# lisqzqng/Video-based-gait-analysis-for-dementia

Hardware: AMD Instinct MI355X
Metric: frames/sec (224x224, seq=16) (higher is better)
Workload: dtype f32

## Files before the change

### video-based-gait-analysis-for-dementia_amd/csrc/conv_pw.hip

```cpp
#include "kernels.h"
#include "device.h"

namespace grk {

namespace {


template <int KC, int NT, int RUN , bool MASK >
__global__ __launch_bounds__(256) __attribute__((amdgpu_waves_per_eu(2))) void conv_pw_f32(const ConvArgs a) {
    constexpr int run = RUN;
    constexpr int KS = KC / 4;
    const int lane = threadIdx.x & 63, l15 = lane & 15, lq = lane >> 4;
    const int HW = a.H * a.W, runs = HW / (16 * run), groups = (a.Cout + 16 * NT - 1) / (16 * NT);
    const int w = blockIdx.x * 4 + (threadIdx.x >> 6);
    if (w >= a.N * runs * groups) return;
    const int g = w % groups, t = w / groups, n = t / runs, px0 = (t - n * runs) * 16 * run, co0 = g * 16 * NT;
    float bw[KS][NT];
#pragma unroll
    for (int s = 0; s < KS; ++s)
#pragma unroll
        for (int nt = 0; nt < NT; ++nt) bw[s][nt] = a.w[(size_t)(4 * s + lq) * a.CoutPad + co0 + nt * 16 + l15];
    float bias[NT];
#pragma unroll
    for (int nt = 0; nt < NT; ++nt) bias[nt] = a.bias[co0 + nt * 16 + l15];
    const float* inp = a.in + ((size_t)n * a.in_ctot + a.in_coff + lq) * HW + px0 + l15;
    float* outp = a.out + ((size_t)n * a.out_ctot + a.out_coff + co0 + l15) * HW + px0 + 4 * lq;
    const float* addp = a.n_add ? a.add[0] + ((size_t)n * a.add_ctot[0] + a.add_coff[0] + co0 + l15) * HW + px0 + 4 * lq : nullptr;
    const size_t cstr = (size_t)16 * HW;
    float cur[KS], nxt[KS];
#pragma unroll
    for (int s = 0; s < KS; ++s) cur[s] = inp[(size_t)(4 * s) * HW];
    for (int tile = 0; tile < run; ++tile) {
        const int tn = tile + 1 < run ? tile + 1 : tile;
        f32x4 res[NT];
        if (addp) {
#pragma unroll
            for (int nt = 0; nt < NT; ++nt)
                if (!MASK || co0 + nt * 16 + l15 < a.Cout) res[nt] = *reinterpret_cast<const f32x4*>(addp + nt * cstr + 16 * tile);
        }
#pragma unroll
        for (int s = 0; s < KS; ++s) nxt[s] = inp[(size_t)(4 * s) * HW + 16 * tn];
        f32x4 acc[NT];
#pragma unroll
        for (int nt = 0; nt < NT; ++nt) acc[nt] = f32x4{0.f, 0.f, 0.f, 0.f};
#pragma unroll
        for (int s = 0; s < KS; ++s)
#pragma unroll
            for (int nt = 0; nt < NT; ++nt) acc[nt] = __builtin_amdgcn_mfma_f32_16x16x4f32(cur[s], bw[s][nt], acc[nt], 0, 0, 0);
#pragma unroll
        for (int nt = 0; nt < NT; ++nt) {
            f32x4 v = acc[nt] + bias[nt];
            if (addp) v += res[nt];
            if (a.relu) {
#pragma unroll
                for (int r = 0; r < 4; ++r) v[r] = fmaxf(v[r], 0.f);
            }
            if (!MASK || co0 + nt * 16 + l15 < a.Cout) *reinterpret_cast<f32x4*>(outp + nt * cstr + 16 * tile) = v;
        }
#pragma unroll
        for (int s = 0; s < KS; ++s) cur[s] = nxt[s];
    }
}

}

bool conv_pw_eligible(int cin, int cout, int ks, int stride, int h, int w, int n_add) {
    return ks == 1 && stride == 1 && n_add <= 1 && (h * w) % (16 * 14) == 0 && ((cin == 64 && cout >= 17) || (cin == 128 && cout >= 17 && cout <= 32));
}

hipError_t launch_conv_pw(ConvArgs a, hipStream_t s) {
    if (!conv_pw_eligible(a.Cin, a.Cout, a.ks, a.stride, a.H, a.W, a.n_add) || (a.n_add == 1 && a.add_shift[0] != 0) || a.CinPad < a.Cin)
        return hipErrorInvalidValue;
    const int nt = a.Cout > 32 ? 4 : 2, groups = (a.Cout + 16 * nt - 1) / (16 * nt), tiles = a.H * a.W / 16;
    if (a.CoutPad < groups * 16 * nt) return hipErrorInvalidValue;
    if (tiles % 14 != 0 || tiles % 2 != 0) return hipErrorInvalidValue;
    const bool lng = (long)a.N * (tiles / 14) * groups >= 800;
    const dim3 grid((a.N * (tiles / (lng ? 14 : 2)) * groups + 3) / 4);
    const bool mask = a.Cout % (16 * nt) != 0;
#define GRK_PW2(KC, NT, RUN) (mask ? launch_k(conv_pw_f32<KC, NT, RUN, true>, grid, dim3(256), 0, s, a) : launch_k(conv_pw_f32<KC, NT, RUN, false>, grid, dim3(256), 0, s, a))
#define GRK_PW(KC, NT) (lng ? GRK_PW2(KC, NT, 14) : GRK_PW2(KC, NT, 2))
    if (a.Cin == 64) return nt == 4 ? GRK_PW(64, 4) : GRK_PW(64, 2);
    return GRK_PW(128, 2);
#undef GRK_PW2
#undef GRK_PW
}

}
```

### video-based-gait-analysis-for-dementia_amd/csrc/conv_stem.hip

```cpp
#include "kernels.h"
#include "device.h"

namespace grk {

namespace {

__global__ __launch_bounds__(256) void conv_stem_f32(const ConvArgs a) {
    const int lane = threadIdx.x & 63, l15 = lane & 15, lq = lane >> 4;
    const int row = blockIdx.x * 4 + (threadIdx.x >> 6);
    if (row >= a.N * a.Ho) return;
    const int n = row / a.Ho, y = row - n * a.Ho;
    const float* w = a.w;
    float bw[7][4];
#pragma unroll
    for (int s = 0; s < 7; ++s)
#pragma unroll
        for (int nt = 0; nt < 4; ++nt) bw[s][nt] = w[(s * 4 + nt) * 64 + lane];
    float bias[4];
#pragma unroll
    for (int nt = 0; nt < 4; ++nt) bias[nt] = a.bias[nt * 16 + l15];
    const float* rowp[7];
    int kxm1[7];
    bool yok[7];
    const float* inb = a.in + ((size_t)n * a.in_ctot + a.in_coff) * a.H * a.W;
#pragma unroll
    for (int s = 0; s < 7; ++s) {
        const int k = 4 * s + lq, kk = k < 27 ? k : 26, c = kk / 9, t = kk - 9 * c, ky = t / 3, kx = t - 3 * ky;
        const int yin = 2 * y + ky - 1;
        yok[s] = yin >= 0 && yin < a.H;
        rowp[s] = inb + ((size_t)c * a.H + (yok[s] ? yin : 0)) * a.W;
        kxm1[s] = kx - 1;
    }
    auto fetch = [&](int x0, float (&v)[7]) {
#pragma unroll
        for (int s = 0; s < 7; ++s) {
            const int xi = 2 * (x0 + l15) + kxm1[s];
            const bool ok = yok[s] && xi >= 0 && xi < a.W;
            const float t = rowp[s][ok ? xi : 0];
            v[s] = ok ? t : 0.f;
        }
    };
    float cur[7], nxt[7];
    fetch(0, cur);
    float* ob = a.out + (((size_t)n * a.out_ctot + a.out_coff + l15) * a.Ho + y) * a.Wo + 4 * lq;
    const size_t cstride = (size_t)16 * a.Ho * a.Wo;
    for (int x0 = 0; x0 < a.Wo; x0 += 16) {
        fetch(x0 + 16 < a.Wo ? x0 + 16 : x0, nxt);
        f32x4 acc[4];
#pragma unroll
        for (int nt = 0; nt < 4; ++nt) acc[nt] = f32x4{0.f, 0.f, 0.f, 0.f};
#pragma unroll
        for (int s = 0; s < 7; ++s)
#pragma unroll
            for (int nt = 0; nt < 4; ++nt) acc[nt] = __builtin_amdgcn_mfma_f32_16x16x4f32(cur[s], bw[s][nt], acc[nt], 0, 0, 0);
#pragma unroll
        for (int nt = 0; nt < 4; ++nt) {
            f32x4 v = acc[nt] + bias[nt];
            if (a.relu) {
#pragma unroll
                for (int r = 0; r < 4; ++r) v[r] = fmaxf(v[r], 0.f);
            }
            *reinterpret_cast<f32x4*>(ob + nt * cstride + x0) = v;
        }
#pragma unroll
        for (int s = 0; s < 7; ++s) cur[s] = nxt[s];
    }
}

}

bool conv_stem_eligible(int cin, int cout, int ks, int stride, int h, int w, int n_add) {
    return cin == 3 && cout == 64 && ks == 3 && stride == 2 && n_add == 0 && h % 2 == 0 && w % 32 == 0;
}

void pack_stem_weights(const double* w_folded , float* out ) {
    for (int s = 0; s < 7; ++s)
        for (int nt = 0; nt < 4; ++nt)
            for (int lq = 0; lq < 4; ++lq)
                for (int l15 = 0; l15 < 16; ++l15) {
                    const int k = 4 * s + lq, co = 16 * nt + l15;
                    out[(s * 4 + nt) * 64 + lq * 16 + l15] = k < 27 ? (float)w_folded[(size_t)co * 27 + k] : 0.f;
                }
}

hipError_t launch_conv_stem(ConvArgs a, hipStream_t s) {
    if (!conv_stem_eligible(a.Cin, a.Cout, a.ks, a.stride, a.H, a.W, a.n_add) || a.Ho * 2 != a.H || a.Wo * 2 != a.W) return hipErrorInvalidValue;
    const int rows = a.N * a.Ho;
    return launch_k(conv_stem_f32, dim3((rows + 3) / 4), dim3(256), 0, s, a);
}

}
```

### video-based-gait-analysis-for-dementia_amd/csrc/grnet_run.cpp

```cpp
#include "grnet_impl.h"

namespace grk { thread_local GraphRecorder* g_recorder = nullptr; }

int grnet::allocate() {
    if (plan_arena(compact, arena_plan)) return fail(GRNET_ESTATE, "the activation arena could not be planned: a launch group or the assignment violates the sharing rule");
    const size_t total = (size_t)arena_plan.total;
    arena_floats = total;
    void* q = nullptr;
    if (hipMalloc(&q, total * sizeof(float)) != hipSuccess)
        return fail(GRNET_ENOMEM, std::string("hipMalloc of the ") + (compact ? "compact " : "") + "activation arena (" + std::to_string(total * 4 >> 20) + " MiB) failed");
    arena = static_cast<float*>(q);
    if (hipMemset(arena, 0, 64 * sizeof(float)) != hipSuccess) return fail(GRNET_EHIP, "hipMemset failed");
    zeros = arena;
    if (hipEventCreateWithFlags(&ev_fork, hipEventDisableTiming) != hipSuccess) return fail(GRNET_EHIP, "hipEventCreate failed");
    if (int rc = install_schedule(max_frames)) return rc;
    if (hipStreamCreateWithFlags(&capture_stream, hipStreamNonBlocking) != hipSuccess) return fail(GRNET_EHIP, "hipStreamCreate failed");
    const size_t n = max_frames;
    int rc;
    if ((rc = dev_alloc(&d_plf, n * 128 * 24))) return rc;
    if ((rc = dev_alloc(&d_csf, n * 64 * 24))) return rc;
    if ((rc = dev_alloc(&d_stats, softmax_pool_ws_floats((int)n)))) return rc;
    if ((rc = dev_alloc(&d_rot6d, n * 144))) return rc;
    if ((rc = dev_alloc(&d_shape, n * 10))) return rc;
    if ((rc = dev_alloc(&d_cam, n * 3))) return rc;
// ... 258 lines not shown
            src.w = fp.w_dev[i][j - i - 1];
        }
    }
    HIP_TRY(dtype == 1 ? launch_hr_fuse_up_bf16(a, s) : launch_hr_fuse_up(a, s));
    return 0;
}

grnet::HeadOutputs grnet::head_outputs(const grnet_outputs_t& o) const {
    return {o.pred_rot6d ? o.pred_rot6d : d_rot6d, o.rotmat ? o.rotmat : d_rotmat, o.theta ? o.theta : d_theta,
            o.verts ? o.verts : d_verts,           o.kp_3d ? o.kp_3d : d_kp3d,     o.kp_2d ? o.kp_2d : d_kp2d};
}

int grnet::enqueue(const float* frames, int n, const grnet_outputs_t& o, hipStream_t s, bool convs_only) {
    int launches = 0;
    last_n = n;
    float* plf = o.point_local_feat ? o.point_local_feat : d_plf;
    float* csf = o.cam_shape_feats ? o.cam_shape_feats : d_csf;
    const auto [rot6d, rotmat, theta, verts, kp3d, kp2d] = head_outputs(o);
    const std::vector<Op>& ops = ops_flat;
    const std::vector<hipEvent_t>& op_events = op_events_flat;
    GraphRecorder* rec = g_recorder;
    const bool lanes = multi_lane && !rec;
    std::vector<hipGraphNode_t> lane_last(kLanes, nullptr), op_node(rec ? ops.size() : 0, nullptr);
    hipStream_t lane_stream[kLanes];
    for (int l = 0; l < kLanes; ++l) lane_stream[l] = s;
    if (lanes) {
        HIP_TRY(hipEventRecord(ev_fork, s));
        for (int l = 1; l < lanes_used; ++l) {
            lane_stream[l] = side[l];
            HIP_TRY(hipStreamWaitEvent(side[l], ev_fork, 0));
        }
    }
    hipStream_t caller = s;
    for (size_t oi = 0; oi < ops.size(); ++oi) {
        const Op& op = ops[oi];
        if (convs_only && op.kind != Op::CONV && op.kind != Op::FUSEUP) continue;
        s = lane_stream[op.lane];
        const int lane = multi_lane ? op.lane : 0;
        if (lanes)
            for (int w : op.waits) HIP_TRY(hipStreamWaitEvent(s, op_events[w], 0));
        if (tl_start && !rec) HIP_TRY(hipEventRecord((*tl_start)[oi], s));
        if (rec) {
            rec->deps.clear();
            rec->n_chain = lane_last[lane] ? 1 : 0;
            if (lane_last[lane]) rec->deps.push_back(lane_last[lane]);
            if (multi_lane)
                for (int w : op.waits)
                    if (op_node[w] && std::find(rec->deps.begin(), rec->deps.end(), op_node[w]) == rec->deps.end()) rec->deps.push_back(op_node[w]);
        }
        static const char* abl_skip = GRNET_AB_STR(ABL_SKIP);
        if (abl_skip && (op.kind == Op::CONV || op.kind == Op::FUSEUP)) {
            const std::string lbl = op_label(op);
            bool skip = false;
            for (const char* q = abl_skip; *q;) {
                const char* e = strchr(q, ',');
                const std::string pat = e ? std::string(q, e) : std::string(q);
                if (!pat.empty() && lbl.find(pat) != std::string::npos) skip = true;
                q = e ? e + 1 : q + strlen(q);
            }
            if (skip) {
                if (tl_end && !rec) HIP_TRY(hipEventRecord((*tl_end)[oi], s));
                if (lanes && op.record) HIP_TRY(hipEventRecord(op_events[oi], s));
                continue;
            }
        }
        switch (op.kind) {
// ... 9 lines not shown
            }
            case Op::SUM: {
                const auto& sv = sum_views[op.conv_idx];
                SumArgs a = op.sum;
                a.N = n;
                bind(sv.out, a.out, a.out_ctot, a.out_coff);
                for (int k = 0; k < a.n_add; ++k) {
                    bind(sv.adds[k].v, a.add[k], a.add_ctot[k], a.add_coff[k]);
                    a.add_shift[k] = sv.adds[k].shift;
                }
                if (dtype == 1) HIP_TRY(launch_fuse_sum_bf16(a, s));
                else HIP_TRY(launch_fuse_sum(a, s));
                ++launches;
                break;
            }
            case Op::FUSEUP:
                if (int rc = launch_fuse_up_op(fuse_ups[op.conv_idx], n, s)) return rc;
                ++launches;
                break;
            case Op::BILINEAR:
                if (dtype == 1) HIP_TRY(launch_bilinear2x_bf16(base(op.bin), base(op.bout), n, op.bin.c, op.bin.h, op.bin.w, s));
                else HIP_TRY(launch_bilinear2x(base(op.bin), base(op.bout), n, op.bin.c, op.bin.h, op.bin.w, s));
                ++launches;
                break;
            case Op::POOL:
                if (dtype == 1)
                    HIP_TRY(launch_softmax_pool_bf16(base(v_heat), v_heat.ctot, bf16_at(v_smpl_feats), 128, v_smpl_feats.ctot, bf16_at(v_csmap), 64,
                                                     v_csmap.ctot, d_stats, n, 56 * 56, s));
                else
                    HIP_TRY(launch_softmax_pool(base(v_heat), 25, base(v_smpl_feats), 128, base(v_csmap), 64, plf, csf, d_stats, n, 56 * 56, s));
                ++launches;
                break;
            case Op::TAIL:
                HIP_TRY(launch_head_tail(d_stats, true, plf, csf, tailw, rot6d, d_shape, d_cam, rotmat, theta, n, s));
                ++launches;
                break;
            case Op::SMPL:
                HIP_TRY(launch_smpl(d_shape, rotmat, d_cam, smpl, d_A, verts, kp3d, kp2d, n, s));
                launches += 4;
                break;
        }
        if (tl_end && !rec) HIP_TRY(hipEventRecord((*tl_end)[oi], s));
        if (lanes && op.record) HIP_TRY(hipEventRecord(op_events[oi], s));
        if (rec && !rec->deps.empty()) lane_last[lane] = op_node[oi] = rec->deps[0];
    }
    s = caller;
    if (lanes)
        for (int l = 1; l < lanes_used; ++l) {
            HIP_TRY(hipEventRecord(ev_join[l], side[l]));
            HIP_TRY(hipStreamWaitEvent(s, ev_join[l], 0));
        }
    if (!convs_only) {
        auto copy_out = [&](float* dst, const float* src, size_t bytes) -> int {
            if (!dst) return 0;
            if (!rec) { HIP_TRY(hipMemcpyAsync(dst, src, bytes, hipMemcpyDeviceToDevice, s)); return 0; }
            std::vector<hipGraphNode_t> deps;
            for (hipGraphNode_t nd : lane_last) if (nd) deps.push_back(nd);
            hipGraphNode_t node = nullptr;
            HIP_TRY(hipGraphAddMemcpyNode1D(&node, rec->graph, deps.data(), deps.size(), dst, src, bytes, hipMemcpyDeviceToDevice));
            return 0;
        };
        int rc;
        if (dtype == 1) {
            auto conv_out = [&](float* dst, const View& v) -> int {
                if (!dst) return 0;
                if (rec) {
                    rec->deps.clear();
                    for (hipGraphNode_t nd : lane_last) if (nd) rec->deps.push_back(nd);
                }
                HIP_TRY(launch_nhwc_bf16_to_nchw_f32(base(v), dst, n, v.c, v.h, v.w, v.ctot, v.coff, s));
                return 0;
            };
// ... 297 lines not shown
```

### video-based-gait-analysis-for-dementia_amd/csrc/head_kernels.hip

```cpp
#include "kernels.h"
#include "device.h"

namespace grk {

__global__ __launch_bounds__(256) void fuse_sum_kernel(const SumArgs a) {
    const int HW = a.H * a.W, n = blockIdx.x / a.C, c = blockIdx.x - n * a.C;
    const float inv_w = 1.0f / (float)a.W;
    for (int pix = threadIdx.x * 4; pix < HW; pix += 1024) {
        f32x4 v = f32x4{0.f, 0.f, 0.f, 0.f};
        for (int k = 0; k < a.n_add; ++k) {
            const int sh = a.add_shift[k];
            if (sh == 0) {
                v += *reinterpret_cast<const f32x4*>(a.add[k] + ((size_t)n * a.add_ctot[k] + a.add_coff[k] + c) * HW + pix);
            } else {
                const int hs = a.H >> sh, ws = a.W >> sh;
                const float* ap = a.add[k] + ((size_t)n * a.add_ctot[k] + a.add_coff[k] + c) * (hs * ws);
#pragma unroll
                for (int r = 0; r < 4; ++r) {
                    const int y = (int)(((float)(pix + r) + 0.5f) * inv_w), x = (pix + r) - y * a.W;
                    v[r] += ap[(y >> sh) * ws + (x >> sh)];
                }
            }
        }
        if (a.relu) {
// ... 286 lines not shown
    const float ux = a2x - d * b1x, uy = a2y - d * b1y, uz = a2z - d * b1z;
    const float n2 = fmaxf(sqrtf(ux * ux + uy * uy + uz * uz), 1e-6f);
    const float b2x = ux / n2, b2y = uy / n2, b2z = uz / n2;
    const float b3x = b1y * b2z - b1z * b2y, b3y = b1z * b2x - b1x * b2z, b3z = b1x * b2y - b1y * b2x;
    R[0] = b1x; R[1] = b2x; R[2] = b3x;
    R[3] = b1y; R[4] = b2y; R[5] = b3y;
    R[6] = b1z; R[7] = b2z; R[8] = b3z;
}

__device__ __forceinline__ void rotmat_to_aa_dev(const float* R, float* aa) {
    const float m00 = R[0], m01 = R[3], m02 = R[6];
    const float m10 = R[1], m11 = R[4], m12 = R[7];
    const float m20 = R[2], m21 = R[5], m22 = R[8];
    float q0, q1, q2, q3, t;
    if (m22 < 1e-6f) {
        if (m00 > m11) { t = 1.f + m00 - m11 - m22; q0 = m12 - m21; q1 = t; q2 = m01 + m10; q3 = m20 + m02; }
        else           { t = 1.f - m00 + m11 - m22; q0 = m20 - m02; q1 = m01 + m10; q2 = t; q3 = m12 + m21; }
    } else {
        if (m00 < -m11) { t = 1.f - m00 - m11 + m22; q0 = m01 - m10; q1 = m20 + m02; q2 = m12 + m21; q3 = t; }
        else            { t = 1.f + m00 + m11 + m22; q0 = t; q1 = m12 - m21; q2 = m20 - m02; q3 = m01 - m10; }
    }
    const float sc = 0.5f / sqrtf(t);
    q0 *= sc; q1 *= sc; q2 *= sc; q3 *= sc;
    const float s2 = q1 * q1 + q2 * q2 + q3 * q3;
    const float sn = sqrtf(s2);
    const float two_theta = 2.f * (q0 < 0.f ? atan2f(-sn, -q0) : atan2f(sn, q0));
    const float k = s2 > 0.f ? two_theta / sn : 2.f;
    float a0 = q1 * k, a1 = q2 * k, a2 = q3 * k;
    aa[0] = isnan(a0) ? 0.f : a0;
    aa[1] = isnan(a1) ? 0.f : a1;
    aa[2] = isnan(a2) ? 0.f : a2;
}

template <bool FROM_PARTS>
__global__ __launch_bounds__(256) void head_tail_kernel(const float* __restrict__ part, const float* __restrict__ zstats, float* __restrict__ plf, float* __restrict__ csf, TailWeights w,
                                                          float* __restrict__ rot6d, float* __restrict__ shape,
                                                          float* __restrict__ cam, float* __restrict__ rotmat,
                                                          float* __restrict__ theta) {
    __shared__ float s_plf[128 * 24];
    __shared__ __align__(16) float s_csf[64 * 24];
    __shared__ float s_pose[24 * 6];
    __shared__ float s_sc[13];
    __shared__ float s_pp[4][144];
    __shared__ float s_sp[13][8];
    __shared__ float s_zw[kPoolSplit + 1][24];
    const int n = blockIdx.x, tid = threadIdx.x;
    if constexpr (FROM_PARTS) {
        if (tid < 24) {
            float m[kPoolSplit], sm[kPoolSplit], M = -INFINITY, S = 0.f;
#pragma unroll
            for (int z = 0; z < kPoolSplit; ++z) {
                m[z] = zstats ? zstats[(((size_t)n * kPoolSplit + z) * 24 + tid) * 2] : 0.f;
                sm[z] = zstats ? zstats[(((size_t)n * kPoolSplit + z) * 24 + tid) * 2 + 1] : 0.f;
                M = fmaxf(M, m[z]);
            }
#pragma unroll
            for (int z = 0; z < kPoolSplit; ++z) {
                const float wz = zstats ? expf(m[z] - M) : 1.f;
                s_zw[z][tid] = wz;
                S += sm[z] * wz;
            }
            s_zw[kPoolSplit][tid] = zstats ? 1.f / S : 1.f;
        }
        __syncthreads();
    }
    static_assert((192 * 24) % (256 * 6) == 0, "partials loop");
    if constexpr (!FROM_PARTS) {
        for (int e = tid; e < 128 * 24; e += 256) s_plf[e] = plf[(size_t)n * 128 * 24 + e];
        for (int e = tid; e < 64 * 24; e += 256) s_csf[e] = csf[(size_t)n * 64 * 24 + e];
    } else
    for (int e0 = tid; e0 < 192 * 24; e0 += 256 * 6) {
        float v[6][kPoolSplit];
#pragma unroll
        for (int u = 0; u < 6; ++u)
#pragma unroll
            for (int sp = 0; sp < kPoolSplit; ++sp) v[u][sp] = part[((size_t)n * kPoolSplit + sp) * (192 * 24) + e0 + u * 256];
#pragma unroll
        for (int u = 0; u < 6; ++u) {
            const int e = e0 + u * 256;
            const int j = e % 24;
            float acc = 0.f;
#pragma unroll
            for (int sp = 0; sp < kPoolSplit; ++sp) acc += v[u][sp] * s_zw[sp][j];
            acc *= s_zw[kPoolSplit][j];
            if (e < 128 * 24) { s_plf[e] = acc; plf[(size_t)n * 128 * 24 + e] = acc; }
            else { s_csf[e - 128 * 24] = acc; csf[(size_t)n * 64 * 24 + e - 128 * 24] = acc; }
        }
    }
    __syncthreads();
    if (tid < 144) {
        const int g = tid % 36, cq = tid / 36;
        const f32x4* wp = reinterpret_cast<const f32x4*>(w.pose_w) + (size_t)(cq * 32) * 36 + g;
        const float* pl = s_plf + cq * 32 * 24;
        const int ja = (4 * g) / 6, jb = (4 * g + 1) / 6, jc = (4 * g + 2) / 6, jd = (4 * g + 3) / 6;
        f32x4 acc = {0.f, 0.f, 0.f, 0.f};
#pragma unroll 16
        for (int c = 0; c < 32; ++c) {
            const f32x4 wv = wp[c * 36];
            acc[0] += pl[c * 24 + ja] * wv[0];
            acc[1] += pl[c * 24 + jb] * wv[1];
            acc[2] += pl[c * 24 + jc] * wv[2];
            acc[3] += pl[c * 24 + jd] * wv[3];
        }
#pragma unroll
// ... 13 lines not shown
    __syncthreads();
    if (tid < 144) {
        const float acc = (s_pp[0][tid] + s_pp[1][tid]) + (s_pp[2][tid] + s_pp[3][tid]);
        s_pose[tid] = acc;
        rot6d[(size_t)n * 144 + tid] = acc;
    } else if (tid < 157) {
        const int o = tid - 144;
        float acc = 0.f;
#pragma unroll
        for (int seg = 0; seg < 8; ++seg) acc += s_sp[o][seg];
        s_sc[o] = acc + (o < 10 ? w.shape_b[o] : w.cam_b[o - 10]);
    }
    __syncthreads();
    if (tid < 24) {
        float R[9], aa[3];
        rot6d_to_rotmat_dev(&s_pose[tid * 6], R);
#pragma unroll
        for (int k = 0; k < 9; ++k) rotmat[(size_t)n * 216 + tid * 9 + k] = R[k];
        rotmat_to_aa_dev(R, aa);
        theta[(size_t)n * 85 + 3 + tid * 3 + 0] = aa[0];
        theta[(size_t)n * 85 + 3 + tid * 3 + 1] = aa[1];
        theta[(size_t)n * 85 + 3 + tid * 3 + 2] = aa[2];
    }
    if (tid >= 64 && tid < 74) {
        const int o = tid - 64;
        shape[(size_t)n * 10 + o] = s_sc[o];
        theta[(size_t)n * 85 + 75 + o] = s_sc[o];
    }
    if (tid >= 128 && tid < 131) {
        const int o = tid - 128;
        cam[(size_t)n * 3 + o] = s_sc[10 + o];
        theta[(size_t)n * 85 + o] = s_sc[10 + o];
    }
}

hipError_t launch_head_tail(const float* pool_ws, bool range_stats, float* plf, float* csf, TailWeights w, float* rot6d, float* shape, float* cam,
                            float* rotmat, float* theta, int N, hipStream_t s) {
    GRK_TRY(launch_k(head_tail_kernel<true>, dim3(N), dim3(256), 0, s, pool_ws + (size_t)N * kPoolStatsFloats, range_stats ? pool_ws : (const float*)nullptr, plf, csf,
                     w, rot6d, shape, cam, rotmat, theta));
    return hipGetLastError();
}

hipError_t launch_head_tail_from_feats(const float* plf, const float* csf, TailWeights w, float* rot6d, float* shape, float* cam, float* rotmat,
                                       float* theta, int N, hipStream_t s) {
    GRK_TRY(launch_k(head_tail_kernel<false>, dim3(N), dim3(256), 0, s, (const float*)nullptr, (const float*)nullptr, const_cast<float*>(plf), const_cast<float*>(csf), w,
                     rot6d, shape, cam, rotmat, theta));
    return hipGetLastError();
}

__global__ __launch_bounds__(256) void rot6d_to_rotmat_kernel(const float* __restrict__ x, float* __restrict__ R, int m) {
    const int i = blockIdx.x * 256 + threadIdx.x;
    if (i >= m) return;
    float xi[6], r[9];
#pragma unroll
    for (int k = 0; k < 6; ++k) xi[k] = x[(size_t)i * 6 + k];
    rot6d_to_rotmat_dev(xi, r);
#pragma unroll
    for (int k = 0; k < 9; ++k) R[(size_t)i * 9 + k] = r[k];
}
__global__ __launch_bounds__(256) void rotmat_to_aa_kernel(const float* __restrict__ R, float* __restrict__ aa, int m) {
    const int i = blockIdx.x * 256 + threadIdx.x;
    if (i >= m) return;
    float r[9], a[3];
#pragma unroll
    for (int k = 0; k < 9; ++k) r[k] = R[(size_t)i * 9 + k];
    rotmat_to_aa_dev(r, a);
#pragma unroll
    for (int k = 0; k < 3; ++k) aa[(size_t)i * 3 + k] = a[k];
}
hipError_t launch_rot6d_to_rotmat(const float* x, float* R, int m, hipStream_t s) {
    GRK_TRY(launch_k(rot6d_to_rotmat_kernel, dim3((m + 255) / 256), dim3(256), 0, s, x, R, m));
    return hipGetLastError();
}
hipError_t launch_rotmat_to_aa(const float* R, float* aa, int m, hipStream_t s) {
    GRK_TRY(launch_k(rotmat_to_aa_kernel, dim3((m + 255) / 256), dim3(256), 0, s, R, aa, m));
    return hipGetLastError();
}

__global__ __launch_bounds__(320) void smpl_chain_kernel(const float* __restrict__ betas, const float* __restrict__ rotmat, SmplTables t,
                                                           float* __restrict__ A_ws, float* __restrict__ kp3d, float* __restrict__ feat) {
    __shared__ float J[24][3];
    __shared__ float G[24][12];
    __shared__ float Rs[216];
    __shared__ int par[24], depth[24];
    const int n = blockIdx.x, tid = threadIdx.x;
    for (int e = tid; e < 216; e += 320) Rs[e] = rotmat[(size_t)n * 216 + e];
    if (tid < 24) par[tid] = t.parents[tid];
    for (int e = tid; e < 72; e += 320) {
        float v = t.J_template[e];
#pragma unroll
        for (int l = 0; l < 10; ++l) v += t.J_shapedirs[e * 10 + l] * betas[(size_t)n * 10 + l];
        J[e / 3][e % 3] = v;
    }
    for (int e = tid; e < kBlendK; e += 320) {
        float v = 0.f;
        if (e < 207) v = rotmat[(size_t)n * 216 + 9 + e] - ((e % 9 == 0 || e % 9 == 4 || e % 9 == 8) ? 1.f : 0.f);
        else if (e < 217) v = betas[(size_t)n * 10 + e - 207];
        else if (e == 217) v = 1.f;
        feat[(size_t)n * kBlendK + e] = v;
    }
    __syncthreads();
    if (tid < 24) {
        int d = 0;
        for (int p = par[tid]; p >= 0 && d < 24; p = par[p]) ++d;
        depth[tid] = d;
    }
    __syncthreads();
    const int ji = tid / 12, rc = tid - ji * 12, r = rc >> 2, c = rc & 3;
    const bool mine = tid < 288;
    const int myd = mine ? depth[ji] : -1, p = mine ? par[ji] : 0;
    for (int d = 0; d < 24; ++d) {
        if (mine && myd == d) {
            if (d == 0) {
                G[ji][rc] = c < 3 ? Rs[ji * 9 + r * 3 + c] : J[ji][r];
            } else {
                const float g0 = G[p][r * 4 + 0], g1 = G[p][r * 4 + 1], g2 = G[p][r * 4 + 2];
                if (c < 3) {
                    const float* Ri = Rs + ji * 9;
                    G[ji][rc] = g0 * Ri[c] + g1 * Ri[3 + c] + g2 * Ri[6 + c];
                } else {
                    const float t0 = J[ji][0] - J[p][0], t1 = J[ji][1] - J[p][1], t2 = J[ji][2] - J[p][2];
                    G[ji][rc] = g0 * t0 + g1 * t1 + g2 * t2 + G[p][r * 4 + 3];
                }
            }
        }
        __syncthreads();
        if (d >= 1 && __syncthreads_count(mine && myd > d) == 0) break;
    }
    for (int e = tid; e < 24 * 12; e += 320) {
        const int i = e / 12, rc2 = e % 12, r2 = rc2 / 4, c2 = rc2 % 4;
        float v = G[i][rc2];
        if (c2 == 3) {
            kp3d[((size_t)n * 29 + i) * 3 + r2] = v;
            v -= G[i][r2 * 4 + 0] * J[i][0] + G[i][r2 * 4 + 1] * J[i][1] + G[i][r2 * 4 + 2] * J[i][2];
        }
        A_ws[(size_t)n * 288 + e] = v;
    }
}

constexpr int kNumVerts = 6890;
constexpr int kBlendCols = kNumVerts * 3;

template <int MT>
__device__ __forceinline__ void blend_pass(const float* __restrict__ As, const float (&bv)[kBlendK / 4], float* __restrict__ Cs, int l15, int lq, int wave) {
    constexpr int LD = kBlendK + 1, KS = kBlendK / 4;
    f32x4 acc[MT];
#pragma unroll
    for (int m = 0; m < MT; ++m) acc[m] = f32x4{0.f, 0.f, 0.f, 0.f};
    const float* a0 = As + l15 * LD + lq;
#pragma unroll
    for (int ks = 0; ks < KS; ++ks)
#pragma unroll
        for (int m = 0; m < MT; ++m) acc[m] = __builtin_amdgcn_mfma_f32_16x16x4f32(a0[m * 16 * LD + 4 * ks], bv[ks], acc[m], 0, 0, 0);
#pragma unroll
    for (int m = 0; m < MT; ++m)
#pragma unroll
        for (int r = 0; r < 4; ++r) Cs[(m * 16 + lq * 4 + r) * 64 + wave * 16 + l15] = acc[m][r];
}

__global__ __launch_bounds__(256, 2) void smpl_blend_mfma_kernel(const float* __restrict__ feat, const float* __restrict__ blend, float* __restrict__ vposed,
                                                               int N) {
    constexpr int LD = kBlendK + 1, KS = kBlendK / 4;
    __shared__ float As[64 * LD];
    __shared__ __align__(16) float Cs[64 * 64];
    const int tid = threadIdx.x, lane = tid & 63, wave = tid >> 6, l15 = lane & 15, lq = lane >> 4;
    const int col = blockIdx.x * 64 + wave * 16 + l15;
    const bool cok = col < kBlendCols;
    const float* bp = blend + (cok ? col : 0) + (size_t)lq * kBlendCols;
    float bv[KS];
#pragma unroll
// ... 63 lines not shown
                                                            float* __restrict__ kp3d, float* __restrict__ kp2d) {
    __shared__ float red[4][3];
    __shared__ float sj[29][3];
    const int n = blockIdx.x, tid = threadIdx.x, lane = tid & 63, wave = tid >> 6;
    const float* vn = verts + (size_t)n * kNumVerts * 3;
    float a0 = 0.f, a1 = 0.f, a2 = 0.f;
    for (int k = tid; k < t.thorax_n; k += 256) {
        const int v = t.thorax_idx[k];
        const float w = t.thorax_w[k];
        a0 += w * vn[v * 3]; a1 += w * vn[v * 3 + 1]; a2 += w * vn[v * 3 + 2];
    }
    a0 = wave_sum(a0); a1 = wave_sum(a1); a2 = wave_sum(a2);
    if (lane == 0) { red[wave][0] = a0; red[wave][1] = a1; red[wave][2] = a2; }
    if (tid < 72) sj[tid / 3][tid % 3] = kp3d[(size_t)n * 87 + tid];
    if (tid >= 96 && tid < 108) {
        const int e = tid - 96, jj = e / 3, d = e % 3;
        const int vid = jj == 0 ? 2746 : jj == 1 ? 2445 : jj == 2 ? 6191 : 5905;
        sj[24 + jj][d] = vn[vid * 3 + d];
    }
    __syncthreads();
    if (tid < 3) sj[28][tid] = red[0][tid] + red[1][tid] + red[2][tid] + red[3][tid];
    __syncthreads();
    if (tid < 87) kp3d[(size_t)n * 87 + tid] = sj[tid / 3][tid % 3];
    if (tid < 29 && cam != nullptr && kp2d != nullptr) {
        const float s = cam[(size_t)n * 3], tx = cam[(size_t)n * 3 + 1], ty = cam[(size_t)n * 3 + 2];
        const float tz = 2.f * 5000.f / (224.f * s + 1e-9f);
        const float X = sj[tid][0] + tx, Y = sj[tid][1] + ty, Z = sj[tid][2] + tz;
        kp2d[((size_t)n * 29 + tid) * 2 + 0] = 5000.f * (X / Z) / 112.f;
        kp2d[((size_t)n * 29 + tid) * 2 + 1] = 5000.f * (Y / Z) / 112.f;
    }
}

hipError_t launch_smpl(const float* betas, const float* rotmat, const float* cam, SmplTables t, float* A_ws, float* verts,
                       float* kp3d, float* kp2d, int N, hipStream_t s) {
    float* feat = A_ws + (size_t)N * 288;
    GRK_TRY(launch_k(smpl_chain_kernel, dim3(N), dim3(320), 0, s, betas, rotmat, t, A_ws, kp3d, feat));
    GRK_TRY(launch_k(smpl_blend_mfma_kernel, dim3((kBlendCols + 63) / 64), dim3(256), 0, s, (const float*)feat, t.blend, verts, N));
    GRK_TRY(launch_k(smpl_skin_kernel, dim3((kNumVerts + 255) / 256, N), dim3(256), 0, s, t, (const float*)A_ws, verts));
    GRK_TRY(launch_k(smpl_joints_kernel, dim3(N), dim3(256), 0, s, verts, cam, t, kp3d, kp2d));
    return hipGetLastError();
}

}
```

### video-based-gait-analysis-for-dementia_amd/csrc/kernels.h

```cpp
#pragma once
#include <hip/hip_runtime.h>
#include <stdint.h>

#include <initializer_list>
#include <mutex>
#include <string>
#include <tuple>
#include <utility>
#include <vector>

#ifdef GRNET_ABLATION
#include <cstdlib>
#define GRNET_AB(name, dflt) (getenv("GRNET_" #name) ? atoi(getenv("GRNET_" #name)) : (dflt))
#define GRNET_AB_F(name, dflt) (getenv("GRNET_" #name) ? atof(getenv("GRNET_" #name)) : (dflt))
#define GRNET_AB_SET(name) (getenv("GRNET_" #name) != nullptr)
#define GRNET_AB_STR(name) getenv("GRNET_" #name)
#else
#define GRNET_AB(name, dflt) (dflt)
#define GRNET_AB_F(name, dflt) (dflt)
#define GRNET_AB_SET(name) false
#define GRNET_AB_STR(name) (static_cast<const char*>(nullptr))
#endif

#define GRK_TRY(expr) do { hipError_t _e = (expr); if (_e != hipSuccess) return _e; } while (0)
// ... 179 lines not shown
    const float* shape_b;
    const float* cam_w;
    const float* cam_b;
};
hipError_t launch_head_tail(const float* pool_ws, bool range_stats , float* plf, float* csf, TailWeights w, float* rot6d, float* shape, float* cam,
                            float* rotmat, float* theta, int N, hipStream_t s);
hipError_t launch_head_tail_from_feats(const float* plf, const float* csf, TailWeights w, float* rot6d, float* shape, float* cam, float* rotmat,
                                       float* theta, int N, hipStream_t s);
hipError_t launch_rot6d_to_rotmat(const float* x, float* R, int m, hipStream_t s);
hipError_t launch_rotmat_to_aa(const float* R, float* aa, int m, hipStream_t s);
size_t softmax_pool_ws_floats(int N);
constexpr int kPoolStatsFloats = 7 * 24 * 2;
constexpr int kPoolSplit = 7;

constexpr int kBlendK = 220;
constexpr int kSmplWsFloatsPerFrame = 288 + kBlendK;
struct SmplTables {
    const float* blend;
    const int* skin_idx;
    const float* skin_w;
    int skin_k;
    const float* J_template;
    const float* J_shapedirs;
    const float* lbs_weights;
    const int* thorax_idx;
    const float* thorax_w;
    int thorax_n;
    const int* parents;
    int extra_ptr[10];
    const int* extra_idx;
    const float* extra_w;
};
hipError_t launch_smpl(const float* betas, const float* rotmat, const float* cam, SmplTables t, float* A_ws,
                       float* verts, float* kp3d, float* kp2d, int N, hipStream_t s);

constexpr int kOneEuroBlock = 32;
struct OneEuroCoef { float a_d, one_minus_a_d, two_pi, min_cutoff, beta; };
hipError_t launch_one_euro(const float* x, int ld, int T, OneEuroCoef c, float* xhat, hipStream_t s);
hipError_t launch_aa_to_rotmat(const float* aa, float* R, int m, const float* betas0, float* betas_out, int nb, hipStream_t s);
int smooth_joint_count(int kind);
hipError_t launch_smpl_joints54(const float* kp29, const float* verts, SmplTables t, int kind, float* joints, int n, hipStream_t s);

constexpr int kJregMaxRows = 64;
constexpr int kJregSlices = 27;
constexpr int kJregChunks = 16;
size_t joint_regress_pack_floats(int jout);
size_t joint_regress_workspace_floats(int jout, int max_frames);
void joint_regress_pack(const float* W , int jout, float* out );
hipError_t launch_joint_regress(const float* verts, const float* wpack, int jout, float* partial, float* joints, int n, hipStream_t s);

constexpr int kRasterSlots = 16;
constexpr int kRasterMaxDim = 4096;
constexpr int kRasterSnapBits = 8;
constexpr int kRasterCoordLimit = 1 << 28;
struct RasterView { float M[9]; int H, W; };
struct RasterMesh {
    const int* faces;
    const int* vf_off;
    const int* vf_idx;
    int n_verts, n_faces;
};
struct RasterWork {
    float* q;
    int* xy;
    float* z;
    float* nrm;
    int* bbox;
// ... 115 lines not shown
```

Measured before the change: 4535.

## Rebalance pointwise conv runs, split stem rows across waves, fuse SMPL chain into head

The pointwise conv now chooses its run length from the CU count and lets runs cross frame boundaries, so small batches fill the GPU. Uneven splits are absorbed by an extra tile on some waves. The stem conv splits each output row into parts of 7 tiles per wave, loading all inputs before the MFMAs instead of looping over the whole row. The SMPL kinematic chain is folded into the head tail kernel, which runs with 320 threads, removing one launch at the cost of a larger block and more instantiations.

```diff
diff --git a/video-based-gait-analysis-for-dementia_amd/csrc/conv_pw.hip b/video-based-gait-analysis-for-dementia_amd/csrc/conv_pw.hip
--- a/video-based-gait-analysis-for-dementia_amd/csrc/conv_pw.hip
+++ b/video-based-gait-analysis-for-dementia_amd/csrc/conv_pw.hip
@@ -1,3 +1,4 @@
+#include <algorithm>
 #include "kernels.h"
 #include "device.h"
 
@@ -7,14 +8,15 @@
 
 
 template <int KC, int NT, int RUN , bool MASK >
-__global__ __launch_bounds__(256) __attribute__((amdgpu_waves_per_eu(2))) void conv_pw_f32(const ConvArgs a) {
-    constexpr int run = RUN;
-    constexpr int KS = KC / 4;
+__global__ __launch_bounds__(256) __attribute__((amdgpu_waves_per_eu(2))) void conv_pw_f32(const ConvArgs a, const int n_runs, const int extra) {
+    constexpr int KS = KC / 4, PF = 1;
     const int lane = threadIdx.x & 63, l15 = lane & 15, lq = lane >> 4;
-    const int HW = a.H * a.W, runs = HW / (16 * run), groups = (a.Cout + 16 * NT - 1) / (16 * NT);
-    const int w = blockIdx.x * 4 + (threadIdx.x >> 6);
-    if (w >= a.N * runs * groups) return;
-    const int g = w % groups, t = w / groups, n = t / runs, px0 = (t - n * runs) * 16 * run, co0 = g * 16 * NT;
+    const int HW = a.H * a.W, tpf = HW / 16, groups = (a.Cout + 16 * NT - 1) / (16 * NT);
+    const int w = blockIdx.x * 4 + __builtin_amdgcn_readfirstlane(threadIdx.x >> 6);
+    const int g = w % groups, r = w / groups;
+    if (r >= n_runs) return;
+    const int len = RUN + (r < extra ? 1 : 0), T0 = r * RUN + (r < extra ? r : extra);
+    const int n = T0 / tpf, t0 = T0 - n * tpf, cross = tpf - t0, px0 = t0 * 16, co0 = g * 16 * NT;
     float bw[KS][NT];
 #pragma unroll
     for (int s = 0; s < KS; ++s)
@@ -26,40 +28,54 @@
     const float* inp = a.in + ((size_t)n * a.in_ctot + a.in_coff + lq) * HW + px0 + l15;
     float* outp = a.out + ((size_t)n * a.out_ctot + a.out_coff + co0 + l15) * HW + px0 + 4 * lq;
     const float* addp = a.n_add ? a.add[0] + ((size_t)n * a.add_ctot[0] + a.add_coff[0] + co0 + l15) * HW + px0 + 4 * lq : nullptr;
+    const long seam_in = (long)(a.in_ctot - 1) * HW, seam_out = (long)(a.out_ctot - 1) * HW, seam_add = a.n_add ? (long)(a.add_ctot[0] - 1) * HW : 0;
+    auto off = [&](int i, long seam) { return (long)16 * i + (i >= cross ? seam : 0); };
     const size_t cstr = (size_t)16 * HW;
-    float cur[KS], nxt[KS];
+    float buf[PF + 1][KS];
 #pragma unroll
-    for (int s = 0; s < KS; ++s) cur[s] = inp[(size_t)(4 * s) * HW];
-    for (int tile = 0; tile < run; ++tile) {
-        const int tn = tile + 1 < run ? tile + 1 : tile;
+    for (int p = 0; p < PF; ++p) {
+        const long o = off(p < len ? p : len - 1, seam_in);
+#pragma unroll
+        for (int s = 0; s < KS; ++s) buf[p][s] = inp[(size_t)(4 * s) * HW + o];
+    }
+    auto tile_step = [&](const int tile, const bool ahead) {
         f32x4 res[NT];
         if (addp) {
+            const long o = off(tile, seam_add);
 #pragma unroll
             for (int nt = 0; nt < NT; ++nt)
-                if (!MASK || co0 + nt * 16 + l15 < a.Cout) res[nt] = *reinterpret_cast<const f32x4*>(addp + nt * cstr + 16 * tile);
+                if (!MASK || co0 + nt * 16 + l15 < a.Cout) res[nt] = *reinterpret_cast<const f32x4*>(addp + nt * cstr + o);
         }
+        if (ahead) {
+            const long o = off(tile + PF < len ? tile + PF : len - 1, seam_in);
 #pragma unroll
-        for (int s = 0; s < KS; ++s) nxt[s] = inp[(size_t)(4 * s) * HW + 16 * tn];
+            for (int s = 0; s < KS; ++s) buf[PF][s] = inp[(size_t)(4 * s) * HW + o];
+        }
         f32x4 acc[NT];
 #pragma unroll
         for (int nt = 0; nt < NT; ++nt) acc[nt] = f32x4{0.f, 0.f, 0.f, 0.f};
 #pragma unroll
         for (int s = 0; s < KS; ++s)
 #pragma unroll
-            for (int nt = 0; nt < NT; ++nt) acc[nt] = __builtin_amdgcn_mfma_f32_16x16x4f32(cur[s], bw[s][nt], acc[nt], 0, 0, 0);
+            for (int nt = 0; nt < NT; ++nt) acc[nt] = __builtin_amdgcn_mfma_f32_16x16x4f32(buf[0][s], bw[s][nt], acc[nt], 0, 0, 0);
+        const long oo = off(tile, seam_out);
 #pragma unroll
         for (int nt = 0; nt < NT; ++nt) {
             f32x4 v = acc[nt] + bias[nt];
             if (addp) v += res[nt];
             if (a.relu) {
 #pragma unroll
-                for (int r = 0; r < 4; ++r) v[r] = fmaxf(v[r], 0.f);
+                for (int r4 = 0; r4 < 4; ++r4) v[r4] = fmaxf(v[r4], 0.f);
             }
-            if (!MASK || co0 + nt * 16 + l15 < a.Cout) *reinterpret_cast<f32x4*>(outp + nt * cstr + 16 * tile) = v;
+            if (!MASK || co0 + nt * 16 + l15 < a.Cout) *reinterpret_cast<f32x4*>(outp + nt * cstr + oo) = v;
         }
 #pragma unroll
-        for (int s = 0; s < KS; ++s) cur[s] = nxt[s];
-    }
+        for (int p = 0; p < PF; ++p)
+#pragma unroll
+            for (int s = 0; s < KS; ++s) buf[p][s] = buf[p + 1][s];
+    };
+    for (int tile = 0; tile < RUN; ++tile) tile_step(tile, true);
+    if (len > RUN) tile_step(RUN, false);
 }
 
 }
@@ -68,17 +84,47 @@
     return ks == 1 && stride == 1 && n_add <= 1 && (h * w) % (16 * 14) == 0 && ((cin == 64 && cout >= 17) || (cin == 128 && cout >= 17 && cout <= 32));
 }
 
+static void conv_pw_form(long tiles, int groups, int cus, int* run, int* n_runs, int* extra) {
+    const long slots = std::max(1, 4 * cus / groups);
+    if (tiles >= 14 * slots) { *run = 14; *n_runs = (int)(tiles / 14); *extra = 0; return; }
+    *n_runs = (int)std::min(slots, tiles);
+    *run = (int)(tiles / *n_runs);
+    *extra = (int)(tiles - (long)*run * *n_runs);
+}
+
 hipError_t launch_conv_pw(ConvArgs a, hipStream_t s) {
     if (!conv_pw_eligible(a.Cin, a.Cout, a.ks, a.stride, a.H, a.W, a.n_add) || (a.n_add == 1 && a.add_shift[0] != 0) || a.CinPad < a.Cin)
         return hipErrorInvalidValue;
-    const int nt = a.Cout > 32 ? 4 : 2, groups = (a.Cout + 16 * nt - 1) / (16 * nt), tiles = a.H * a.W / 16;
+    const int nt = a.Cout > 32 ? 4 : 2, groups = (a.Cout + 16 * nt - 1) / (16 * nt), tpf = a.H * a.W / 16;
     if (a.CoutPad < groups * 16 * nt) return hipErrorInvalidValue;
-    if (tiles % 14 != 0 || tiles % 2 != 0) return hipErrorInvalidValue;
-    const bool lng = (long)a.N * (tiles / 14) * groups >= 800;
-    const dim3 grid((a.N * (tiles / (lng ? 14 : 2)) * groups + 3) / 4);
+    if (tpf % 14 != 0) return hipErrorInvalidValue;
+    const long tiles = (long)a.N * tpf;
+    int cus = 0, run = 0, n_runs = 0, extra = 0;
+    if (hipError_t e = device_cu_count(&cus); e != hipSuccess) return e;
+    conv_pw_form(tiles, groups, cus, &run, &n_runs, &extra);
+#ifdef GRNET_ABLATION
+    static const int code = GRNET_AB(PW_FORM, 0);
+    if (code) {
+        extra = 0;
+        if (code == 99) run = tiles / 14 * groups >= 800 ? 14 : 2;
+        else if (code % 10 || code == 10) run = code;
+        else {
+            n_runs = std::max(1, code * 1024 / 10 / groups);
+            run = (int)(tiles / n_runs);
+            extra = (int)(tiles - (long)run * n_runs);
+        }
+        if (code == 99 || code % 10 || code == 10) { if (tiles % run) return hipErrorInvalidValue; n_runs = (int)(tiles / run); }
+        if (run < 1 || run > 14 || (extra && run + 1 > tpf)) return hipErrorInvalidValue;
+    }
+#endif
+    const dim3 grid((n_runs * groups + 3) / 4);
     const bool mask = a.Cout % (16 * nt) != 0;
-#define GRK_PW2(KC, NT, RUN) (mask ? launch_k(conv_pw_f32<KC, NT, RUN, true>, grid, dim3(256), 0, s, a) : launch_k(conv_pw_f32<KC, NT, RUN, false>, grid, dim3(256), 0, s, a))
-#define GRK_PW(KC, NT) (lng ? GRK_PW2(KC, NT, 14) : GRK_PW2(KC, NT, 2))
+#define GRK_PW2(KC, NT, RUN) (mask ? launch_k(conv_pw_f32<KC, NT, RUN, true>, grid, dim3(256), 0, s, a, n_runs, extra) : launch_k(conv_pw_f32<KC, NT, RUN, false>, grid, dim3(256), 0, s, a, n_runs, extra))
+#define GRK_PW(KC, NT)                                                                                                                           \
+    (run == 14 ? GRK_PW2(KC, NT, 14) : run == 13 ? GRK_PW2(KC, NT, 13) : run == 12 ? GRK_PW2(KC, NT, 12) : run == 11 ? GRK_PW2(KC, NT, 11) :       \
+     run == 10 ? GRK_PW2(KC, NT, 10) : run == 9 ? GRK_PW2(KC, NT, 9) : run == 8 ? GRK_PW2(KC, NT, 8) : run == 7 ? GRK_PW2(KC, NT, 7) :             \
+     run == 6 ? GRK_PW2(KC, NT, 6) : run == 5 ? GRK_PW2(KC, NT, 5) : run == 4 ? GRK_PW2(KC, NT, 4) : run == 3 ? GRK_PW2(KC, NT, 3) :               \
+     run == 2 ? GRK_PW2(KC, NT, 2) : run == 1 ? GRK_PW2(KC, NT, 1) : hipErrorInvalidValue)
     if (a.Cin == 64) return nt == 4 ? GRK_PW(64, 4) : GRK_PW(64, 2);
     return GRK_PW(128, 2);
 #undef GRK_PW2
diff --git a/video-based-gait-analysis-for-dementia_amd/csrc/conv_stem.hip b/video-based-gait-analysis-for-dementia_amd/csrc/conv_stem.hip
--- a/video-based-gait-analysis-for-dementia_amd/csrc/conv_stem.hip
+++ b/video-based-gait-analysis-for-dementia_amd/csrc/conv_stem.hip
@@ -5,20 +5,13 @@
 
 namespace {
 
-__global__ __launch_bounds__(256) void conv_stem_f32(const ConvArgs a) {
+template <int TPW >
+__global__ __launch_bounds__(256) void conv_stem_f32(const ConvArgs a, const int parts ) {
     const int lane = threadIdx.x & 63, l15 = lane & 15, lq = lane >> 4;
-    const int row = blockIdx.x * 4 + (threadIdx.x >> 6);
-    if (row >= a.N * a.Ho) return;
+    const int wv = blockIdx.x * 4 + __builtin_amdgcn_readfirstlane(threadIdx.x >> 6);
+    if (wv >= a.N * a.Ho * parts) return;
+    const int row = wv / parts, xb = (wv - row * parts) * (16 * TPW);
     const int n = row / a.Ho, y = row - n * a.Ho;
-    const float* w = a.w;
-    float bw[7][4];
-#pragma unroll
-    for (int s = 0; s < 7; ++s)
-#pragma unroll
-        for (int nt = 0; nt < 4; ++nt) bw[s][nt] = w[(s * 4 + nt) * 64 + lane];
-    float bias[4];
-#pragma unroll
-    for (int nt = 0; nt < 4; ++nt) bias[nt] = a.bias[nt * 16 + l15];
     const float* rowp[7];
     int kxm1[7];
     bool yok[7];
@@ -31,39 +24,52 @@
         rowp[s] = inb + ((size_t)c * a.H + (yok[s] ? yin : 0)) * a.W;
         kxm1[s] = kx - 1;
     }
-    auto fetch = [&](int x0, float (&v)[7]) {
+    float v[TPW][7];
 #pragma unroll
-        for (int s = 0; s < 7; ++s) {
-            const int xi = 2 * (x0 + l15) + kxm1[s];
-            const bool ok = yok[s] && xi >= 0 && xi < a.W;
-            const float t = rowp[s][ok ? xi : 0];
-            v[s] = ok ? t : 0.f;
+    for (int t = 0; t < TPW; ++t) {
+        const int x0 = xb + 16 * t;
+        if (x0 < a.Wo) {
+#pragma unroll
+            for (int s = 0; s < 7; ++s) {
+                const int xi = 2 * (x0 + l15) + kxm1[s];
+                const bool ok = yok[s] && xi >= 0 && xi < a.W;
+                const float q = rowp[s][ok ? xi : 0];
+                v[t][s] = ok ? q : 0.f;
+            }
         }
-    };
-    float cur[7], nxt[7];
-    fetch(0, cur);
+    }
+    const float* w = a.w;
+    float bw[7][4];
+#pragma unroll
+    for (int s = 0; s < 7; ++s)
+#pragma unroll
+        for (int nt = 0; nt < 4; ++nt) bw[s][nt] = w[(s * 4 + nt) * 64 + lane];
+    float bias[4];
+#pragma unroll
+    for (int nt = 0; nt < 4; ++nt) bias[nt] = a.bias[nt * 16 + l15];
     float* ob = a.out + (((size_t)n * a.out_ctot + a.out_coff + l15) * a.Ho + y) * a.Wo + 4 * lq;
     const size_t cstride = (size_t)16 * a.Ho * a.Wo;
-    for (int x0 = 0; x0 < a.Wo; x0 += 16) {
-        fetch(x0 + 16 < a.Wo ? x0 + 16 : x0, nxt);
-        f32x4 acc[4];
 #pragma unroll
-        for (int nt = 0; nt < 4; ++nt) acc[nt] = f32x4{0.f, 0.f, 0.f, 0.f};
+    for (int t = 0; t < TPW; ++t) {
+        const int x0 = xb + 16 * t;
+        if (x0 < a.Wo) {
+            f32x4 acc[4];
 #pragma unroll
-        for (int s = 0; s < 7; ++s)
+            for (int nt = 0; nt < 4; ++nt) acc[nt] = f32x4{0.f, 0.f, 0.f, 0.f};
 #pragma unroll
-            for (int nt = 0; nt < 4; ++nt) acc[nt] = __builtin_amdgcn_mfma_f32_16x16x4f32(cur[s], bw[s][nt], acc[nt], 0, 0, 0);
+            for (int s = 0; s < 7; ++s)
 #pragma unroll
-        for (int nt = 0; nt < 4; ++nt) {
-            f32x4 v = acc[nt] + bias[nt];
-            if (a.relu) {
+                for (int nt = 0; nt < 4; ++nt) acc[nt] = __builtin_amdgcn_mfma_f32_16x16x4f32(v[t][s], bw[s][nt], acc[nt], 0, 0, 0);
 #pragma unroll
-                for (int r = 0; r < 4; ++r) v[r] = fmaxf(v[r], 0.f);
+            for (int nt = 0; nt < 4; ++nt) {
+                f32x4 o = acc[nt] + bias[nt];
+                if (a.relu) {
+#pragma unroll
+                    for (int r = 0; r < 4; ++r) o[r] = fmaxf(o[r], 0.f);
+                }
+                *reinterpret_cast<f32x4*>(ob + nt * cstride + x0) = o;
             }
-            *reinterpret_cast<f32x4*>(ob + nt * cstride + x0) = v;
         }
-#pragma unroll
-        for (int s = 0; s < 7; ++s) cur[s] = nxt[s];
     }
 }
 
@@ -85,8 +91,24 @@
 
 hipError_t launch_conv_stem(ConvArgs a, hipStream_t s) {
     if (!conv_stem_eligible(a.Cin, a.Cout, a.ks, a.stride, a.H, a.W, a.n_add) || a.Ho * 2 != a.H || a.Wo * 2 != a.W) return hipErrorInvalidValue;
-    const int rows = a.N * a.Ho;
-    return launch_k(conv_stem_f32, dim3((rows + 3) / 4), dim3(256), 0, s, a);
+    const int tiles = a.Wo / 16;
+#ifdef GRNET_ABLATION
+    static const int tpw = GRNET_AB(STEM_FORM, 7);
+#else
+    constexpr int tpw = 7;
+#endif
+    const int parts = (tiles + tpw - 1) / tpw;
+    const dim3 grid((a.N * a.Ho * parts + 3) / 4);
+#ifdef GRNET_ABLATION
+    switch (tpw) {
+        case 4: return launch_k(conv_stem_f32<4>, grid, dim3(256), 0, s, a, parts);
+        case 2: return launch_k(conv_stem_f32<2>, grid, dim3(256), 0, s, a, parts);
+        case 1: return launch_k(conv_stem_f32<1>, grid, dim3(256), 0, s, a, parts);
+        case 7: break;
+        default: return hipErrorInvalidValue;
+    }
+#endif
+    return launch_k(conv_stem_f32<7>, grid, dim3(256), 0, s, a, parts);
 }
 
 }
diff --git a/video-based-gait-analysis-for-dementia_amd/csrc/grnet_run.cpp b/video-based-gait-analysis-for-dementia_amd/csrc/grnet_run.cpp
--- a/video-based-gait-analysis-for-dementia_amd/csrc/grnet_run.cpp
+++ b/video-based-gait-analysis-for-dementia_amd/csrc/grnet_run.cpp
@@ -314,6 +314,7 @@
         }
     }
     hipStream_t caller = s;
+    bool chain_in_tail = false;
     for (size_t oi = 0; oi < ops.size(); ++oi) {
         const Op& op = ops[oi];
         if (convs_only && op.kind != Op::CONV && op.kind != Op::FUSEUP) continue;
@@ -389,12 +390,14 @@
                 ++launches;
                 break;
             case Op::TAIL:
-                HIP_TRY(launch_head_tail(d_stats, true, plf, csf, tailw, rot6d, d_shape, d_cam, rotmat, theta, n, s));
+                chain_in_tail = oi + 1 < ops.size() && ops[oi + 1].kind == Op::SMPL;
+                if (chain_in_tail) HIP_TRY(launch_head_tail_chain(d_stats, true, plf, csf, tailw, rot6d, d_shape, d_cam, rotmat, theta, smpl, d_A, kp3d, n, s));
+                else HIP_TRY(launch_head_tail(d_stats, true, plf, csf, tailw, rot6d, d_shape, d_cam, rotmat, theta, n, s));
                 ++launches;
                 break;
             case Op::SMPL:
-                HIP_TRY(launch_smpl(d_shape, rotmat, d_cam, smpl, d_A, verts, kp3d, kp2d, n, s));
-                launches += 4;
+                HIP_TRY(launch_smpl(d_shape, rotmat, d_cam, smpl, d_A, verts, kp3d, kp2d, n, s, chain_in_tail));
+                launches += chain_in_tail ? 3 : 4;
                 break;
         }
         if (tl_end && !rec) HIP_TRY(hipEventRecord((*tl_end)[oi], s));
diff --git a/video-based-gait-analysis-for-dementia_amd/csrc/head_kernels.hip b/video-based-gait-analysis-for-dementia_amd/csrc/head_kernels.hip
--- a/video-based-gait-analysis-for-dementia_amd/csrc/head_kernels.hip
+++ b/video-based-gait-analysis-for-dementia_amd/csrc/head_kernels.hip
@@ -342,11 +342,15 @@
     aa[2] = isnan(a2) ? 0.f : a2;
 }
 
-template <bool FROM_PARTS>
-__global__ __launch_bounds__(256) void head_tail_kernel(const float* __restrict__ part, const float* __restrict__ zstats, float* __restrict__ plf, float* __restrict__ csf, TailWeights w,
-                                                          float* __restrict__ rot6d, float* __restrict__ shape,
-                                                          float* __restrict__ cam, float* __restrict__ rotmat,
-                                                          float* __restrict__ theta) {
+template <int THREADS>
+__device__ __forceinline__ void smpl_chain_frame(const float* __restrict__ betas, const float* __restrict__ rotmat, const SmplTables& t, float* __restrict__ A_ws,
+                                                 float* __restrict__ kp3d, float* __restrict__ feat, int n, int tid);
+
+template <bool FROM_PARTS, bool CHAIN>
+__global__ __launch_bounds__(CHAIN ? 320 : 256) void head_tail_kernel(const float* __restrict__ part, const float* __restrict__ zstats, float* __restrict__ plf, float* __restrict__ csf, TailWeights w,
+                                                          float* __restrict__ rot6d, float* shape ,
+                                                          float* __restrict__ cam, float* rotmat,
+                                                          float* __restrict__ theta, SmplTables smpl, float* __restrict__ A_ws, float* __restrict__ kp3d) {
     __shared__ float s_plf[128 * 24];
     __shared__ __align__(16) float s_csf[64 * 24];
     __shared__ float s_pose[24 * 6];
@@ -379,7 +383,7 @@
         for (int e = tid; e < 128 * 24; e += 256) s_plf[e] = plf[(size_t)n * 128 * 24 + e];
         for (int e = tid; e < 64 * 24; e += 256) s_csf[e] = csf[(size_t)n * 64 * 24 + e];
     } else
-    for (int e0 = tid; e0 < 192 * 24; e0 += 256 * 6) {
+    for (int e0 = tid < 256 ? tid : 192 * 24; e0 < 192 * 24; e0 += 256 * 6) {
         float v[6][kPoolSplit];
 #pragma unroll
         for (int u = 0; u < 6; ++u)
@@ -459,19 +463,30 @@
         cam[(size_t)n * 3 + o] = s_sc[10 + o];
         theta[(size_t)n * 85 + o] = s_sc[10 + o];
     }
+    if constexpr (CHAIN) {
+        __syncthreads();
+        smpl_chain_frame<320>(shape, rotmat, smpl, A_ws, kp3d, A_ws + (size_t)gridDim.x * 288, n, tid);
+    }
 }
 
 hipError_t launch_head_tail(const float* pool_ws, bool range_stats, float* plf, float* csf, TailWeights w, float* rot6d, float* shape, float* cam,
                             float* rotmat, float* theta, int N, hipStream_t s) {
-    GRK_TRY(launch_k(head_tail_kernel<true>, dim3(N), dim3(256), 0, s, pool_ws + (size_t)N * kPoolStatsFloats, range_stats ? pool_ws : (const float*)nullptr, plf, csf,
-                     w, rot6d, shape, cam, rotmat, theta));
+    GRK_TRY(launch_k(head_tail_kernel<true, false>, dim3(N), dim3(256), 0, s, pool_ws + (size_t)N * kPoolStatsFloats, range_stats ? pool_ws : (const float*)nullptr, plf, csf,
+                     w, rot6d, shape, cam, rotmat, theta, SmplTables{}, (float*)nullptr, (float*)nullptr));
+    return hipGetLastError();
+}
+
+hipError_t launch_head_tail_chain(const float* pool_ws, bool range_stats, float* plf, float* csf, TailWeights w, float* rot6d, float* shape, float* cam,
+                                  float* rotmat, float* theta, SmplTables t, float* A_ws, float* kp3d, int N, hipStream_t s) {
+    GRK_TRY(launch_k(head_tail_kernel<true, true>, dim3(N), dim3(320), 0, s, pool_ws + (size_t)N * kPoolStatsFloats, range_stats ? pool_ws : (const float*)nullptr, plf, csf,
+                     w, rot6d, shape, cam, rotmat, theta, t, A_ws, kp3d));
     return hipGetLastError();
 }
 
 hipError_t launch_head_tail_from_feats(const float* plf, const float* csf, TailWeights w, float* rot6d, float* shape, float* cam, float* rotmat,
                                        float* theta, int N, hipStream_t s) {
-    GRK_TRY(launch_k(head_tail_kernel<false>, dim3(N), dim3(256), 0, s, (const float*)nullptr, (const float*)nullptr, const_cast<float*>(plf), const_cast<float*>(csf), w,
-                     rot6d, shape, cam, rotmat, theta));
+    GRK_TRY(launch_k(head_tail_kernel<false, false>, dim3(N), dim3(256), 0, s, (const float*)nullptr, (const float*)nullptr, const_cast<float*>(plf), const_cast<float*>(csf), w,
+                     rot6d, shape, cam, rotmat, theta, SmplTables{}, (float*)nullptr, (float*)nullptr));
     return hipGetLastError();
 }
 
@@ -504,22 +519,23 @@
     return hipGetLastError();
 }
 
-__global__ __launch_bounds__(320) void smpl_chain_kernel(const float* __restrict__ betas, const float* __restrict__ rotmat, SmplTables t,
-                                                           float* __restrict__ A_ws, float* __restrict__ kp3d, float* __restrict__ feat) {
+template <int THREADS>
+__device__ __forceinline__ void smpl_chain_frame(const float* __restrict__ betas, const float* __restrict__ rotmat, const SmplTables& t, float* __restrict__ A_ws,
+                                                 float* __restrict__ kp3d, float* __restrict__ feat, const int n, const int tid) {
+    static_assert(THREADS >= 288, "a thread per entry of the 24 joints' 3x4 matrices");
     __shared__ float J[24][3];
     __shared__ float G[24][12];
     __shared__ float Rs[216];
     __shared__ int par[24], depth[24];
-    const int n = blockIdx.x, tid = threadIdx.x;
-    for (int e = tid; e < 216; e += 320) Rs[e] = rotmat[(size_t)n * 216 + e];
+    for (int e = tid; e < 216; e += THREADS) Rs[e] = rotmat[(size_t)n * 216 + e];
     if (tid < 24) par[tid] = t.parents[tid];
-    for (int e = tid; e < 72; e += 320) {
+    for (int e = tid; e < 72; e += THREADS) {
         float v = t.J_template[e];
 #pragma unroll
         for (int l = 0; l < 10; ++l) v += t.J_shapedirs[e * 10 + l] * betas[(size_t)n * 10 + l];
         J[e / 3][e % 3] = v;
     }
-    for (int e = tid; e < kBlendK; e += 320) {
+    for (int e = tid; e < kBlendK; e += THREADS) {
         float v = 0.f;
         if (e < 207) v = rotmat[(size_t)n * 216 + 9 + e] - ((e % 9 == 0 || e % 9 == 4 || e % 9 == 8) ? 1.f : 0.f);
         else if (e < 217) v = betas[(size_t)n * 10 + e - 207];
@@ -554,7 +570,7 @@
         __syncthreads();
         if (d >= 1 && __syncthreads_count(mine && myd > d) == 0) break;
     }
-    for (int e = tid; e < 24 * 12; e += 320) {
+    for (int e = tid; e < 24 * 12; e += THREADS) {
         const int i = e / 12, rc2 = e % 12, r2 = rc2 / 4, c2 = rc2 % 4;
         float v = G[i][rc2];
         if (c2 == 3) {
@@ -563,6 +579,11 @@
         }
         A_ws[(size_t)n * 288 + e] = v;
     }
+}
+
+__global__ __launch_bounds__(320) void smpl_chain_kernel(const float* __restrict__ betas, const float* __restrict__ rotmat, SmplTables t,
+                                                           float* __restrict__ A_ws, float* __restrict__ kp3d, float* __restrict__ feat) {
+    smpl_chain_frame<320>(betas, rotmat, t, A_ws, kp3d, feat, blockIdx.x, threadIdx.x);
 }
 
 constexpr int kNumVerts = 6890;
@@ -692,9 +713,9 @@
 }
 
 hipError_t launch_smpl(const float* betas, const float* rotmat, const float* cam, SmplTables t, float* A_ws, float* verts,
-                       float* kp3d, float* kp2d, int N, hipStream_t s) {
+                       float* kp3d, float* kp2d, int N, hipStream_t s, bool chain_done) {
     float* feat = A_ws + (size_t)N * 288;
-    GRK_TRY(launch_k(smpl_chain_kernel, dim3(N), dim3(320), 0, s, betas, rotmat, t, A_ws, kp3d, feat));
+    if (!chain_done) GRK_TRY(launch_k(smpl_chain_kernel, dim3(N), dim3(320), 0, s, betas, rotmat, t, A_ws, kp3d, feat));
     GRK_TRY(launch_k(smpl_blend_mfma_kernel, dim3((kBlendCols + 63) / 64), dim3(256), 0, s, (const float*)feat, t.blend, verts, N));
     GRK_TRY(launch_k(smpl_skin_kernel, dim3((kNumVerts + 255) / 256, N), dim3(256), 0, s, t, (const float*)A_ws, verts));
     GRK_TRY(launch_k(smpl_joints_kernel, dim3(N), dim3(256), 0, s, verts, cam, t, kp3d, kp2d));
diff --git a/video-based-gait-analysis-for-dementia_amd/csrc/kernels.h b/video-based-gait-analysis-for-dementia_amd/csrc/kernels.h
--- a/video-based-gait-analysis-for-dementia_amd/csrc/kernels.h
+++ b/video-based-gait-analysis-for-dementia_amd/csrc/kernels.h
@@ -235,7 +235,9 @@
     const float* extra_w;
 };
 hipError_t launch_smpl(const float* betas, const float* rotmat, const float* cam, SmplTables t, float* A_ws,
-                       float* verts, float* kp3d, float* kp2d, int N, hipStream_t s);
+                       float* verts, float* kp3d, float* kp2d, int N, hipStream_t s, bool chain_done = false);
+hipError_t launch_head_tail_chain(const float* pool_ws, bool range_stats, float* plf, float* csf, TailWeights w, float* rot6d, float* shape, float* cam,
+                                  float* rotmat, float* theta, SmplTables t, float* A_ws, float* kp3d, int N, hipStream_t s);
 
 constexpr int kOneEuroBlock = 32;
 struct OneEuroCoef { float a_d, one_minus_a_d, two_pi, min_cutoff, beta; };
```

After: 4537 (median of 5 runs). Within noise of the previous version (+0.0%).
